# weiji14/deepbedmap

Hardware: NVIDIA B200
Metric: continent inference output Mpx/s (higher is better)
Workload: dtype bf16 (fp32 accumulate, fp32 residual stream)

## Files before the change

### deepbedmap_b200/csrc/common.cuh

```cuda
#pragma once
#include <cuda.h>
#include <cuda_bf16.h>
#include <cuda_runtime.h>
#include <stdint.h>
#include <stdio.h>

#include "../../include/deepbedmap_b200.h"

namespace dbm {

void set_error(const char* fmt, ...);
int check_launch(const char* what);

#define DBM_REQUIRE(cond, ...)            \
  do {                                    \
    if (!(cond)) {                        \
      ::dbm::set_error(__VA_ARGS__);      \
      return DBM_ERR_INVALID;             \
    }                                     \
  } while (0)

#define DBM_CUDA(expr)                                                          \
  do {                                                                          \
    cudaError_t _e = (expr);                                                    \
// ... 59 lines not shown
    if ((++spins & 1023u) != 0) return false;
    const unsigned long long now = globaltimer_ns();
    if (t0 == 0) { t0 = now; return false; }
    return now - t0 > 20000000000ull;
  }
};

__device__ __forceinline__ void mbar_wait(uint64_t* bar, uint32_t parity) {
  uint32_t spins = 0;
  while (!mbar_try_wait(bar, parity)) {
    if (++spins > (1u << 26)) {
      printf("dbm: mbarrier wait timeout block %d thread %d\n", blockIdx.x, threadIdx.x);
      __trap();
    }
  }
}

__device__ __forceinline__ void tma_prefetch_desc(const void* tmap) {
  asm volatile("prefetch.tensormap [%0];" ::"l"(tmap) : "memory");
}
__device__ __forceinline__ void tma_load_4d(void* dst, const void* tmap, uint64_t* bar, int c0, int c1,
                                            int c2, int c3) {
  asm volatile(
      "cp.async.bulk.tensor.4d.shared::cluster.global.tile.mbarrier::complete_tx::bytes "
      "[%0], [%1, {%3, %4, %5, %6}], [%2];" ::"r"(smem_u32(dst)),
      "l"(tmap), "r"(smem_u32(bar)), "r"(c0), "r"(c1), "r"(c2), "r"(c3)
      : "memory");
}
__device__ __forceinline__ void bulk_load(void* dst, const void* src, uint32_t bytes, uint64_t* bar) {
  asm volatile(
      "cp.async.bulk.shared::cluster.global.mbarrier::complete_tx::bytes [%0], [%1], %2, [%3];" ::"r"(
          smem_u32(dst)),
      "l"(src), "r"(bytes), "r"(smem_u32(bar))
      : "memory");
}

template <uint32_t kCols>
__device__ __forceinline__ void tmem_alloc(uint32_t* dst_smem) {
  asm volatile("tcgen05.alloc.cta_group::1.sync.aligned.shared::cta.b32 [%0], %1;" ::"r"(
                   smem_u32(dst_smem)),
               "n"(kCols)
               : "memory");
  asm volatile("tcgen05.relinquish_alloc_permit.cta_group::1.sync.aligned;" ::: "memory");
}
template <uint32_t kCols>
__device__ __forceinline__ void tmem_dealloc(uint32_t taddr) {
  asm volatile("tcgen05.dealloc.cta_group::1.sync.aligned.b32 %0, %1;" ::"r"(taddr), "n"(kCols)
               : "memory");
}
__device__ __forceinline__ void tc_fence_before() {
  asm volatile("tcgen05.fence::before_thread_sync;" ::: "memory");
}
__device__ __forceinline__ void tc_fence_after() {
  asm volatile("tcgen05.fence::after_thread_sync;" ::: "memory");
}
__device__ __forceinline__ void umma_bf16(uint32_t d_tmem, uint64_t adesc, uint64_t bdesc, uint32_t idesc,
                                          uint32_t accumulate) {
  asm volatile(
      "{\n\t.reg .pred p;\n\t"
      "setp.ne.b32 p, %4, 0;\n\t"
      "tcgen05.mma.cta_group::1.kind::f16 [%0], %1, %2, %3, p;\n\t}" ::"r"(d_tmem),
      "l"(adesc), "l"(bdesc), "r"(idesc), "r"(accumulate)
      : "memory");
}
template <uint32_t kAOff, uint32_t kBOff>
__device__ __forceinline__ void umma_bf16_off(uint32_t d_tmem, uint32_t a_lo, uint32_t a_hi, uint32_t b_lo,
                                              uint32_t b_hi, uint32_t idesc, uint32_t accumulate) {
  asm volatile(
      "{\n\t.reg .pred p;\n\t.reg .b32 alo, blo;\n\t.reg .b64 ad, bd;\n\t"
      "setp.ne.b32 p, %6, 0;\n\t"
      "add.u32 alo, %1, %7;\n\t"
      "add.u32 blo, %3, %8;\n\t"
      "mov.b64 ad, {alo, %2};\n\t"
      "mov.b64 bd, {blo, %4};\n\t"
      "tcgen05.mma.cta_group::1.kind::f16 [%0], ad, bd, %5, p;\n\t}" ::"r"(d_tmem),
      "r"(a_lo), "r"(a_hi), "r"(b_lo), "r"(b_hi), "r"(idesc), "r"(accumulate), "n"(kAOff), "n"(kBOff)
      : "memory");
}
__device__ __forceinline__ void umma_commit(uint64_t* bar) {
  asm volatile("tcgen05.commit.cta_group::1.mbarrier::arrive::one.shared::cluster.b64 [%0];" ::"r"(
                   smem_u32(bar))
               : "memory");
}
__device__ __forceinline__ void tmem_ld_32x32b_x32(uint32_t taddr, uint32_t (&r)[32]) {
  asm volatile(
      "tcgen05.ld.sync.aligned.32x32b.x32.b32 "
      "{%0, %1, %2, %3, %4, %5, %6, %7, %8, %9, %10, %11, %12, %13, %14, %15, "
      "%16, %17, %18, %19, %20, %21, %22, %23, %24, %25, %26, %27, %28, %29, %30, %31}, [%32];"
      : "=r"(r[0]), "=r"(r[1]), "=r"(r[2]), "=r"(r[3]), "=r"(r[4]), "=r"(r[5]), "=r"(r[6]), "=r"(r[7]),
        "=r"(r[8]), "=r"(r[9]), "=r"(r[10]), "=r"(r[11]), "=r"(r[12]), "=r"(r[13]), "=r"(r[14]),
        "=r"(r[15]), "=r"(r[16]), "=r"(r[17]), "=r"(r[18]), "=r"(r[19]), "=r"(r[20]), "=r"(r[21]),
        "=r"(r[22]), "=r"(r[23]), "=r"(r[24]), "=r"(r[25]), "=r"(r[26]), "=r"(r[27]), "=r"(r[28]),
        "=r"(r[29]), "=r"(r[30]), "=r"(r[31])
      : "r"(taddr)
      : "memory");
}
__device__ __forceinline__ void tmem_wait_ld() {
  asm volatile("tcgen05.wait::ld.sync.aligned;" ::: "memory");
}

__device__ __forceinline__ bool elect_one_sync() {
  uint32_t pred = 0;
  asm volatile(
      "{\n\t.reg .pred P1;\n\t"
      "elect.sync _|P1, 0xFFFFFFFF;\n\t"
      "@P1 mov.s32 %0, 1;\n\t}"
      : "+r"(pred));
  return pred != 0;
}
__device__ __forceinline__ uint64_t make_desc(uint32_t lo, uint32_t hi) {
  return ((uint64_t)hi << 32) | (uint64_t)lo;
}
__device__ __forceinline__ uint32_t desc_lo(uint32_t saddr, uint32_t lbo_bytes) {
  return ((saddr & 0x3FFFFu) >> 4) | (((lbo_bytes >> 4) & 0x3FFFu) << 16);
}
__host__ __device__ constexpr uint32_t desc_hi(uint32_t sbo_bytes) {
  return ((sbo_bytes >> 4) & 0x3FFFu) | (1u << 14);
}

__device__ __forceinline__ uint64_t umma_desc_kmajor_noswz(uint32_t saddr, uint32_t lbo_bytes,
                                                           uint32_t sbo_bytes) {
  uint64_t d = 0;
  d |= (uint64_t)((saddr & 0x3FFFFu) >> 4);
  d |= (uint64_t)((lbo_bytes >> 4) & 0x3FFF) << 16;
  d |= (uint64_t)((sbo_bytes >> 4) & 0x3FFF) << 32;
  d |= (uint64_t)1 << 46;
  return d;
}
__host__ __device__ constexpr uint32_t umma_idesc_bf16(uint32_t M, uint32_t N) {
  return (1u << 4) | (1u << 7) | (1u << 10) | ((N >> 3) << 17) | ((M >> 4) << 24);
}

}
```

### deepbedmap_b200/csrc/debug_bench.cu

```cuda
#include <utility>

#include "common.cuh"

namespace dbm {

template <int N, int MODE, int IDX>
__device__ __forceinline__ void rate_one(uint32_t d, uint32_t a_lo, uint32_t a_hi, uint32_t b_lo, uint32_t b_hi,
                                         uint32_t idesc) {
  constexpr int tap = IDX % 9, ks = (IDX / 9) % 2, j = IDX / 18;
  constexpr uint32_t a_off = MODE == 0   ? (uint32_t)(((2 * ks) * 18 + tap / 3) * 18 + tap % 3 + 8 * j)
                             : MODE == 1 ? (uint32_t)((2 * ks) * 128 + j * 1024)
                                         : (uint32_t)(ks * 2 + (tap % 3) * 1024);
  constexpr uint32_t b_off = MODE == 2 ? (uint32_t)(ks * 2 + (tap % 2) * (N * 8))
                                       : (uint32_t)(((tap % 3) * 4 + 2 * ks) * (N / 8) * 8);
  umma_bf16_off<a_off, b_off>(d + (uint32_t)(j * N), a_lo, a_hi, b_lo, b_hi, idesc, 1u);
}
template <int N, int MODE, int... IDX>
__device__ __forceinline__ void rate_all(uint32_t d, uint32_t a_lo, uint32_t a_hi, uint32_t b_lo, uint32_t b_hi,
                                         uint32_t idesc, std::integer_sequence<int, IDX...>) {
  (rate_one<N, MODE, IDX>(d, a_lo, a_hi, b_lo, b_hi, idesc), ...);
}

template <int N, int MODE>
__global__ void __launch_bounds__(128, 1) umma_rate_kernel(int iters, long long* out) {
  extern __shared__ uint8_t smem_raw[];
  uint8_t* smem = (uint8_t*)(((uintptr_t)smem_raw + 1023) & ~(uintptr_t)1023);
  __shared__ uint64_t bar;
  __shared__ uint32_t tmem_slot;
  for (int i = threadIdx.x; i < 160 * 1024 / 4; i += blockDim.x) ((uint32_t*)smem)[i] = 0x3c003c00u;
  if (threadIdx.x == 0) {
    mbar_init(&bar, 1);
    fence_mbar_init();
  }
  fence_proxy_async_smem();
  if (threadIdx.x < 32) tmem_alloc<512>(&tmem_slot);
  tc_fence_before();
  __syncthreads();
  tc_fence_after();
  const uint32_t tmem = tmem_slot;
  if (threadIdx.x < 32) {
    constexpr uint32_t idesc = umma_idesc_bf16(128, N);
    const uint32_t a0 = smem_u32(smem), b0 = smem_u32(smem + 96 * 1024);
    uint32_t a_lo, a_hi, b_lo, b_hi;
    if (MODE == 0) {
      a_lo = desc_lo(a0, 5184); a_hi = desc_hi(288);
      b_lo = desc_lo(b0, (N / 8) * 128); b_hi = desc_hi(128);
    } else if (MODE == 1) {
      a_lo = desc_lo(a0, 2048); a_hi = desc_hi(128);
      b_lo = desc_lo(b0, (N / 8) * 128); b_hi = desc_hi(128);
    } else {
      a_lo = desc_lo(a0, 16); a_hi = desc_hi(1024) | (2u << 29);
      b_lo = desc_lo(b0, 16); b_hi = desc_hi(1024) | (2u << 29);
    }
    uint32_t ph = 0;
    const long long t0 = clock64();
    for (int it = 0; it < iters; ++it) {
      if (elect_one_sync()) {
        rate_all<N, MODE>(tmem, a_lo, a_hi, b_lo, b_hi, idesc, std::make_integer_sequence<int, 36>{});
        umma_commit(&bar);
      }
      __syncwarp();
      mbar_wait(&bar, ph);
      ph ^= 1;
    }
    const long long t1 = clock64();
    if (threadIdx.x == 0) out[blockIdx.x] = t1 - t0;
  }
  tc_fence_before();
  __syncthreads();
  if (threadIdx.x < 32) {
    tc_fence_after();
    tmem_dealloc<512>(tmem);
  }
}

template <int N, int MODE>
static int launch_rate(int iters, long long* out, int grid, cudaStream_t st) {
  const int smem = 160 * 1024 + 2048;
  DBM_CUDA(cudaFuncSetAttribute(umma_rate_kernel<N, MODE>, cudaFuncAttributeMaxDynamicSharedMemorySize, smem));
  umma_rate_kernel<N, MODE><<<grid, 128, smem, st>>>(iters, out);
  return check_launch("umma_rate_kernel");
}

}

using namespace dbm;

extern "C" int dbm_debug_umma_rate(int mode, int n, int iters, int per_commit, long long* out_cycles, int grid,
                                   cudaStream_t stream) {
  (void)per_commit;
#define DBM_RATE(NN)                                                         \
  if (n == NN) {                                                             \
    if (mode == 0) return launch_rate<NN, 0>(iters, out_cycles, grid, stream); \
    if (mode == 1) return launch_rate<NN, 1>(iters, out_cycles, grid, stream); \
    if (mode == 2) return launch_rate<NN, 2>(iters, out_cycles, grid, stream); \
  }
  DBM_RATE(32) DBM_RATE(64) DBM_RATE(128) DBM_RATE(256)
#undef DBM_RATE
  set_error("umma_rate: unsupported n=%d mode=%d", n, mode);
  return DBM_ERR_INVALID;
}
```

### deepbedmap_b200/csrc/umma_trunk.cu

```cuda
#include "umma_common.cuh"

namespace dbm {

constexpr int kTrunkThreads = 320;
constexpr int kEpiWarps = 8;
constexpr int kTW = 16, kTH = 32;
constexpr int kHW = kTW + 2, kHH = kTH + 2;
constexpr int kTStages = 5;
constexpr int kTABytes = kHW * kHH * 16 * 2;
constexpr int kTBBytesMax = 9 * 16 * 64 * 2;
constexpr int kMaxTrunkLayers = 512;
constexpr int kTrunkSmem = kTStages * (kTABytes + kTBBytesMax) + 256 + kMaxTrunkLayers * 28 + kEpiWarps * 256 + 1024;

struct TrunkMaps {
  CUtensorMap m[3];
};

template <int COUT>
__device__ __forceinline__ void issue_stage_wide(uint32_t d0, uint32_t a_lo, uint32_t a_hi, uint32_t b_lo,
                                                 uint32_t b_hi, uint32_t acc0) {
  constexpr uint32_t idesc = umma_idesc_bf16(128, COUT);
  constexpr uint32_t kBTap = (uint32_t)(2 * (COUT / 8) * 8);
#pragma unroll 1
  for (uint32_t tap = 0; tap < 9; ++tap) {
    const uint32_t a_tap = a_lo + tap + (tap / 3) * (kHW - 3);
    const uint32_t b_tap = b_lo + tap * kBTap;
    const uint32_t acc = tap != 0 ? 1u : acc0;
    umma_bf16_off<0, 0>(d0, a_tap, a_hi, b_tap, b_hi, idesc, acc);
    umma_bf16_off<8, 0>(d0 + 64, a_tap, a_hi, b_tap, b_hi, idesc, acc);
    umma_bf16_off<16 * kHW, 0>(d0 + 128, a_tap, a_hi, b_tap, b_hi, idesc, acc);
    umma_bf16_off<16 * kHW + 8, 0>(d0 + 192, a_tap, a_hi, b_tap, b_hi, idesc, acc);
  }
}

extern int g_trunk_debug;
extern unsigned long long* g_trunk_prof;

struct TrunkParams {
  const TrunkLayer* layers;
  int num_layers;
  int N, H, W, tiles_x, tiles_y, items_per_layer;
  unsigned int* done;
  unsigned long long* prof;
  int debug;
};

__device__ __forceinline__ unsigned int ld_relaxed_gpu(const unsigned int* p) {
  unsigned int v;
  asm volatile("ld.relaxed.gpu.global.u32 %0, [%1];" : "=r"(v) : "l"(p) : "memory");
  return v;
}
__device__ __forceinline__ void fence_acq_rel_gpu() { asm volatile("fence.acq_rel.gpu;" ::: "memory"); }
__device__ __forceinline__ unsigned int ld_acquire_gpu(const unsigned int* p) {
  unsigned int v;
  asm volatile("ld.acquire.gpu.global.u32 %0, [%1];" : "=r"(v) : "l"(p) : "memory");
  return v;
}
struct F8 {
  float v[8];
};
__device__ __forceinline__ F8 ld_cg_f8(const float* p) {
  F8 r;
  asm volatile("ld.global.cg.v8.f32 {%0,%1,%2,%3,%4,%5,%6,%7}, [%8];"
               : "=f"(r.v[0]), "=f"(r.v[1]), "=f"(r.v[2]), "=f"(r.v[3]), "=f"(r.v[4]), "=f"(r.v[5]), "=f"(r.v[6]),
                 "=f"(r.v[7])
               : "l"(p)
               : "memory");
  return r;
}
__device__ __forceinline__ void st_f8(float* p, float a0, float a1, float a2, float a3, float a4, float a5, float a6,
                                      float a7) {
  asm volatile("st.global.v8.f32 [%0], {%1,%2,%3,%4,%5,%6,%7,%8};" ::"l"(p), "f"(a0), "f"(a1), "f"(a2), "f"(a3),
               "f"(a4), "f"(a5), "f"(a6), "f"(a7)
               : "memory");
}

__device__ __forceinline__ void split_bf16x8(const float* v, uint4& hi, uint4& lo) {
  uint32_t h[4], l[4];
#pragma unroll
  for (int i = 0; i < 4; ++i) {
    const __nv_bfloat162 t = __floats2bfloat162_rn(v[2 * i], v[2 * i + 1]);
    const float2 f = __bfloat1622float2(t);
    const __nv_bfloat162 u = __floats2bfloat162_rn(v[2 * i] - f.x, v[2 * i + 1] - f.y);
    h[i] = *reinterpret_cast<const uint32_t*>(&t);
    l[i] = *reinterpret_cast<const uint32_t*>(&u);
  }
  hi = make_uint4(h[0], h[1], h[2], h[3]);
  lo = make_uint4(l[0], l[1], l[2], l[3]);
}
__device__ __forceinline__ int split_slab(int L) { return ((L >> 1) << 2) + (L & 1); }

struct Cursor {
  int grp = 0, step = 0;
};
struct Sched {
  const int* groups;
  int ng, I, Gd, rounds, bid;
  __device__ __forceinline__ bool next(Cursor& c, int& L, int& unit, int& buf) const {
    while (c.grp < ng) {
      const int e = groups[c.grp];
      const bool pair = (e >> 30) & 1;
      const int nsteps = pair ? 2 * rounds : rounds;
      if (c.step >= nsteps) {
        ++c.grp;
        c.step = 0;
        continue;
      }
      const int t = c.step++;
      int round = t, tail = 0;
      if (pair) {
        if (t == 0) round = 0;
        else if (t == nsteps - 1) { round = rounds - 1; tail = 1; }
        else if (t & 1) round = (t + 1) >> 1;
        else { round = (t >> 1) - 1; tail = 1; }
      }
      int r = bid - (int)(((long)c.grp * I) % Gd);
      if (r < 0) r += Gd;
      unit = round * Gd + r;
      if (unit >= I) continue;
      L = (e & 0x3FFFFFFF) + tail;
      buf = round & 1;
      return true;
    }
    return false;
  }
};

template <bool SPLIT>
__global__ void __launch_bounds__(kTrunkThreads, 1)
umma_trunk_kernel(const __grid_constant__ TrunkMaps maps, const TrunkParams p) {
  extern __shared__ uint8_t smem_raw[];
  uint8_t* smem = (uint8_t*)(((uintptr_t)smem_raw + 1023) & ~(uintptr_t)1023);
  uint8_t* smA = smem;
  uint8_t* smB = smem + kTStages * kTABytes;
  uint64_t* bars = (uint64_t*)(smem + kTStages * (kTABytes + kTBBytesMax));
  uint64_t* full = bars;
  uint64_t* empty = bars + kTStages;
  uint64_t* tfull = bars + 2 * kTStages;
  uint64_t* tempty = bars + 2 * kTStages + 2;
  uint32_t* tmem_slot = (uint32_t*)(bars + 2 * kTStages + 4);
  int* ng_slot = (int*)(tmem_slot + 1);
  int4* linfo = (int4*)(smem + kTStages * (kTABytes + kTBBytesMax) + 256);
  const __nv_bfloat16** lw = (const __nv_bfloat16**)(linfo + kMaxTrunkLayers);
  float* sbias_all = (float*)(lw + kMaxTrunkLayers);
  int* groups = (int*)(sbias_all + kEpiWarps * 64);

  const int warp = threadIdx.x >> 5;
  const int lane = threadIdx.x & 31;

  for (int L = threadIdx.x; L < p.num_layers; L += kTrunkThreads) {
    const TrunkLayer* ly = p.layers + L;
    linfo[L] = make_int4(ly->cin, ly->cout, ly->in_map | (ly->mode << 8), ly->in_cs0);
    lw[L] = ly->wpacked;
  }
  if (threadIdx.x == 0) {
    int ng = 0;
    for (int L = 0; L < p.num_layers; ++L) {
      const int mode = p.layers[L].mode;
      const bool ok = mode == 0 || (mode == 1 && p.layers[L].cout == 64 && L + 1 < p.num_layers &&
                                    p.layers[L + 1].mode == 2 && p.layers[L + 1].cout == 32) ||
                      (mode == 2 && L > 0 && p.layers[L - 1].mode == 1);
      if (!ok) {
        if (blockIdx.x == 0) printf("dbm: trunk pass table entry %d: bad pairing (mode %d)\n", L, mode);
        __trap();
      }
      if (mode == 2) continue;
      groups[ng++] = L | (mode == 1 ? (1 << 30) : 0);
    }
    *ng_slot = ng;
  }
  if (warp == 0 && lane == 0) {
    for (int i = 0; i < 3; ++i) tma_prefetch_desc(&maps.m[i]);
    for (int s = 0; s < kTStages; ++s) {
      mbar_init(&full[s], 1);
      mbar_init(&empty[s], 1);
    }
    for (int b = 0; b < 2; ++b) {
      mbar_init(&tfull[b], 1);
      mbar_init(&tempty[b], kEpiWarps / 2);
    }
    fence_mbar_init();
  }
  if (warp == 1) tmem_alloc<512>(tmem_slot);
  tc_fence_before();
  __syncthreads();
  tc_fence_after();
  const uint32_t tmem_base = *tmem_slot;

  const int I = p.items_per_layer;
  const int per_img = p.tiles_x * p.tiles_y;
  Sched sc;
  sc.groups = groups; sc.ng = *ng_slot; sc.I = I; sc.Gd = (int)gridDim.x; sc.bid = (int)blockIdx.x;
  sc.rounds = (I + sc.Gd - 1) / sc.Gd;
  const unsigned int need = (unsigned)(kEpiWarps / 2);

  if (warp == 0) {
    int s = 0;
    uint32_t ph = 0;
    auto flag_of = [&](int L, int unit) -> const unsigned int* {
      if (L == 0 || lane >= 9) return nullptr;
      const int n = unit / per_img;
      const int r = unit - n * per_img;
      const int ty = r / p.tiles_x, tx = r - ty * p.tiles_x;
      const int ny = ty + lane / 3 - 1, nx = tx + lane % 3 - 1;
      if (ny < 0 || ny >= p.tiles_y || nx < 0 || nx >= p.tiles_x) return nullptr;
      return p.done + (size_t)(L - 1) * I + (size_t)n * per_img + ny * p.tiles_x + nx;
    };
    Cursor cur;
    int L, unit, buf;
    bool have = sc.next(cur, L, unit, buf);
    const unsigned int* f_cur = have ? flag_of(L, unit) : nullptr;
    unsigned int v_cur = f_cur != nullptr ? ld_relaxed_gpu(f_cur) : need;
    while (have) {
      const int n = unit / per_img;
      const int r = unit - n * per_img;
      const int ty = r / p.tiles_x, tx = r - ty * p.tiles_x;
      const int4 li = linfo[L];
      const int cin = li.x, cout = li.y, in_map = li.z & 0xFF, in_cs0 = li.w;
      const __nv_bfloat16* wp = lw[L];
      if (L > 0 && !(p.debug & 1)) {
        if (f_cur != nullptr) {
          SpinGuard guard;
          while (v_cur < need) {
            if (guard.expired()) {
              printf("dbm: trunk dependency timeout layer %d unit %d\n", L, unit);
              __trap();
            }
            __nanosleep(64);
            v_cur = ld_relaxed_gpu(f_cur);
          }
        }
        __syncwarp();
        fence_acq_rel_gpu();
      }
      int Ln, unitn, bufn;
      have = sc.next(cur, Ln, unitn, bufn);
      f_cur = have ? flag_of(Ln, unitn) : nullptr;
      v_cur = f_cur != nullptr ? ld_relaxed_gpu(f_cur) : need;
      const CUtensorMap* tm = &maps.m[in_map];
      const uint32_t b_bytes = (uint32_t)(9 * 16 * 2) * (uint32_t)cout;
      const int num_kc = SPLIT ? 3 * (cin >> 4) : (cin >> 4);
      for (int kc = 0; kc < num_kc; ++kc) {
        int slab = in_cs0 + kc * 2;
        if constexpr (SPLIT) {
          const int c16 = kc / 3, t = kc - 3 * c16;
          slab = 2 * in_cs0 + 4 * c16 + (t == 1 ? 2 : 0);
        }
        mbar_wait(&empty[s], ph ^ 1);
        if (elect_one_sync()) {
          if (p.debug & 4) {
            mbar_arrive(&full[s]);
          } else {
            asm volatile("fence.proxy.async.global;" ::: "memory");
            mbar_arrive_expect_tx(&full[s], (uint32_t)kTABytes + b_bytes);
            tma_load_4d(smA + s * kTABytes, tm, &full[s], (tx * kTW - 1) * 8, ty * kTH - 1, slab,
                        (p.debug & 256) ? 0 : n);
            bulk_load(smB + s * kTBBytesMax, wp + (size_t)kc * (b_bytes / 2), b_bytes, &full[s]);
          }
        }
        __syncwarp();
        if (++s == kTStages) { s = 0; ph ^= 1; }
      }
      L = Ln; unit = unitn; buf = bufn;
    }
  } else if (warp == 1) {
    const uint32_t a_hi = desc_hi(kHW * 16);
    const uint32_t b_hi = desc_hi(128);
    const uint32_t smA_u = smem_u32(smA), smB_u = smem_u32(smB);
    int s = 0;
    uint32_t ph = 0;
    uint32_t use[2] = {0, 0};
    Cursor cur;
    int L, unit, buf;
    while (sc.next(cur, L, unit, buf)) {
      const int4 li = linfo[L];
      const int cin = li.x, cout = li.y, mode = li.z >> 8;
      const int num_kc = SPLIT ? 3 * (cin >> 4) : (cin >> 4);
      const long long t0 = p.prof ? clock64() : 0;
      mbar_wait(&tempty[buf], (use[buf] & 1) ^ 1);
      ++use[buf];
      tc_fence_after();
      const long long t1 = p.prof ? clock64() : 0;
      long long tw = 0;
      const uint32_t d0 = tmem_base + (uint32_t)(buf * 256 + (mode == 2 ? 32 : 0));
      for (int kc = 0; kc < num_kc; ++kc) {
        const long long tw0 = p.prof ? clock64() : 0;
        mbar_wait(&full[s], ph);
        tc_fence_after();
        if (p.prof) tw += clock64() - tw0;
        const uint32_t a_lo = desc_lo(smA_u + s * kTABytes, kHW * kHH * 16);
        const uint32_t acc0 = (kc != 0 || mode == 2) ? 1u : 0u;
        if (cout == 32) {
          const uint32_t b_lo = desc_lo(smB_u + s * kTBBytesMax, 4 * 128);
          if (elect_one_sync()) {
            issue_stage_wide<32>(d0, a_lo, a_hi, b_lo, b_hi, acc0);
            umma_commit(&empty[s]);
            if (kc == num_kc - 1) umma_commit(&tfull[buf]);
          }
        } else {
          const uint32_t b_lo = desc_lo(smB_u + s * kTBBytesMax, 8 * 128);
          if (elect_one_sync()) {
            issue_stage_wide<64>(d0, a_lo, a_hi, b_lo, b_hi, acc0);
            umma_commit(&empty[s]);
            if (kc == num_kc - 1) umma_commit(&tfull[buf]);
          }
        }
        __syncwarp();
        if (++s == kTStages) { s = 0; ph ^= 1; }
      }
      if (p.prof && lane == 0) {
        atomicAdd(p.prof + L * 8 + 0, (unsigned long long)(t1 - t0));
        atomicAdd(p.prof + L * 8 + 1, (unsigned long long)tw);
        atomicAdd(p.prof + L * 8 + 2, (unsigned long long)(clock64() - t0));
        atomicAdd(p.prof + L * 8 + 3, 1ull);
      }
    }
  } else {
    const int q = warp & 3;
    const int grp = (warp - 2) >> 2;
    const int m = 32 * q + lane;
    const int gy = m >> 3, xr = m & 7;
    const bool mem = !(p.debug & 2);
    const bool mem_f32 = mem && !(p.debug & 32), mem_bf16 = mem && !(p.debug & 64), mem_res = mem && !(p.debug & 128);
    const size_t plane = (size_t)p.H * p.W;
    float* sbias = sbias_all + (warp - 2) * 64;
    uint32_t use = 0;
    Cursor cur;
    int L, item, buf;
    while (sc.next(cur, L, item, buf)) {
      if (buf != grp) continue;
      const int n_img = item / per_img;
      const int r = item - n_img * per_img;
      const int n = (p.debug & 256) ? 0 : n_img;
      const int ty = r / p.tiles_x, tx = r - ty * p.tiles_x;
      const TrunkLayer ly = p.layers[L];
      const int y0 = ty * kTH + gy;
      const int x0 = tx * kTW + xr;
      const int nbc = ly.mode == 0 ? (ly.cout >> 5) : 1;
      const int col_off = ly.mode == 2 ? 32 : 0;
      const int nblk = 4 * nbc;
      const int cmain = nbc << 5;
      F8 r1[4], r1n[4];
      if (lane < cmain) sbias[lane] = __ldg(ly.bias + lane);
      if (lane + 32 < cmain) sbias[lane + 32] = __ldg(ly.bias + lane + 32);
      if (L > 0 && (ly.res1 || ly.res2) && !(p.debug & 1)) {
        if (lane == 0) {
          const unsigned int* f = p.done + (size_t)(L - 1) * I + item;
          SpinGuard guard;
          while (ld_acquire_gpu(f) < need) {
            if (guard.expired()) {
              printf("dbm: trunk epilogue dependency timeout layer %d item %d\n", L, item);
              __trap();
            }
            __nanosleep(32);
          }
        }
      }
      __syncwarp();
      auto load_r1 = [&](int b, F8 (&dst)[4]) {
        const int j = nbc == 2 ? (b >> 1) : b;
        const int c0 = (b - j * nbc) << 5;
        const int x = x0 + 8 * (j & 1), y = y0 + 16 * (j >> 1);
        if (ly.res1 != nullptr && mem_res && y < p.H && x < p.W) {
          const float* rp =
              ly.res1 + (((size_t)n * (ly.res1_cs_total >> 1) + (c0 >> 3)) * plane + (size_t)y * p.W + x) * 8;
#pragma unroll
          for (int s8 = 0; s8 < 4; ++s8) dst[s8] = ld_cg_f8(rp + (size_t)s8 * plane * 8);
        }
      };
      load_r1(0, r1);
      const long long e0 = p.prof ? clock64() : 0;
      mbar_wait(&tfull[grp], use & 1);
      ++use;
      tc_fence_after();
      const long long e1 = p.prof ? clock64() : 0;
      long long e2 = 0;
      const bool quick = nbc == 1 && ly.res1 == nullptr && ly.res2 == nullptr && ly.out_f32 == nullptr && !ly.up2 &&
                         ly.out_bf16 != nullptr;
      if (quick) {
        const uint32_t tb = tmem_base + ((uint32_t)(32 * q) << 16) + (uint32_t)(grp * 256 + col_off);
#pragma unroll
        for (int half = 0; half < 2; ++half) {
          uint32_t acc2[2][32];
          tmem_ld_32x32b_x32(tb + (uint32_t)((2 * half) * 64), acc2[0]);
          tmem_ld_32x32b_x32(tb + (uint32_t)((2 * half + 1) * 64), acc2[1]);
          tmem_wait_ld();
          if (half == 1) {
            tc_fence_before();
            __syncwarp();
            if (lane == 0) mbar_arrive(&tempty[grp]);
            if (p.prof) e2 = clock64();
          }
#pragma unroll
          for (int jj = 0; jj < 2; ++jj) {
            const int x = x0 + 8 * jj;
            const int y = y0 + 16 * half;
            if (y < p.H && x < p.W && mem_bf16) {
              const size_t pix = (size_t)y * p.W + x;
#pragma unroll
              for (int s8 = 0; s8 < 4; ++s8) {
                const float4 ba = *reinterpret_cast<const float4*>(sbias + 8 * s8);
                const float4 bb = *reinterpret_cast<const float4*>(sbias + 8 * s8 + 4);
                float v[8] = {__uint_as_float(acc2[jj][8 * s8 + 0]) + ba.x, __uint_as_float(acc2[jj][8 * s8 + 1]) + ba.y,
                              __uint_as_float(acc2[jj][8 * s8 + 2]) + ba.z, __uint_as_float(acc2[jj][8 * s8 + 3]) + ba.w,
                              __uint_as_float(acc2[jj][8 * s8 + 4]) + bb.x, __uint_as_float(acc2[jj][8 * s8 + 5]) + bb.y,
                              __uint_as_float(acc2[jj][8 * s8 + 6]) + bb.z, __uint_as_float(acc2[jj][8 * s8 + 7]) + bb.w};
                if (ly.act) {
#pragma unroll
                  for (int i = 0; i < 8; ++i) v[i] = lrelu(v[i]);
                }
                if constexpr (SPLIT) {
                  uint4 hi, lo;
                  split_bf16x8(v, hi, lo);
                  const size_t cs = (size_t)n * (2 * ly.out_cs_total) + split_slab(ly.out_cs0 + s8);
                  *reinterpret_cast<uint4*>(ly.out_bf16 + (cs * plane + pix) * 8) = hi;
                  *reinterpret_cast<uint4*>(ly.out_bf16 + ((cs + 2) * plane + pix) * 8) = lo;
                  continue;
                }
                uint4 o;
                __nv_bfloat162 t0 = __floats2bfloat162_rn(v[0], v[1]);
                __nv_bfloat162 t1 = __floats2bfloat162_rn(v[2], v[3]);
                __nv_bfloat162 t2 = __floats2bfloat162_rn(v[4], v[5]);
                __nv_bfloat162 t3 = __floats2bfloat162_rn(v[6], v[7]);
                o.x = *reinterpret_cast<uint32_t*>(&t0);
                o.y = *reinterpret_cast<uint32_t*>(&t1);
                o.z = *reinterpret_cast<uint32_t*>(&t2);
                o.w = *reinterpret_cast<uint32_t*>(&t3);
                const size_t cs = (size_t)n * ly.out_cs_total + (ly.out_cs0 + s8);
                *reinterpret_cast<uint4*>(ly.out_bf16 + (cs * plane + pix) * 8) = o;
              }
            }
          }
        }
      } else
      for (int b = 0; b < nblk; ++b) {
        const int j = nbc == 2 ? (b >> 1) : b;
        const int c0 = (b - j * nbc) << 5;
        const int x = x0 + 8 * (j & 1);
        const int y = y0 + 16 * (j >> 1);
        const bool valid = (y < p.H) && (x < p.W);
        const size_t pix = (size_t)y * p.W + x;
        uint32_t acc[32];
        tmem_ld_32x32b_x32(tmem_base + ((uint32_t)(32 * q) << 16) + (uint32_t)(grp * 256 + j * 64 + col_off + c0), acc);
        const bool has1 = ly.res1 != nullptr && valid && mem_res, has2 = ly.res2 != nullptr && valid && mem_res;
        if (b + 1 < nblk) load_r1(b + 1, r1n);
        tmem_wait_ld();
        if (b == nblk - 1) {
          tc_fence_before();
          __syncwarp();
          if (lane == 0) mbar_arrive(&tempty[grp]);
          if (p.prof) e2 = clock64();
        }
        if (valid) {
        float v[32];
#pragma unroll
        for (int i4 = 0; i4 < 8; ++i4) {
          const float4 bb = *reinterpret_cast<const float4*>(sbias + c0 + 4 * i4);
          v[4 * i4 + 0] = __uint_as_float(acc[4 * i4 + 0]) + bb.x;
          v[4 * i4 + 1] = __uint_as_float(acc[4 * i4 + 1]) + bb.y;
          v[4 * i4 + 2] = __uint_as_float(acc[4 * i4 + 2]) + bb.z;
          v[4 * i4 + 3] = __uint_as_float(acc[4 * i4 + 3]) + bb.w;
        }
        if (has1) {
#pragma unroll
          for (int i = 0; i < 32; ++i) v[i] = r1[i >> 3].v[i & 7] + ly.beta * v[i];
        }
        if (has2) {
          const float* rp = ly.res2 + (((size_t)n * 8 + (c0 >> 3)) * plane + pix) * 8;
#pragma unroll
          for (int s8 = 0; s8 < 4; ++s8) {
            const F8 rr = ld_cg_f8(rp + (size_t)s8 * plane * 8);
#pragma unroll
            for (int i = 0; i < 8; ++i) v[8 * s8 + i] = rr.v[i] + ly.beta * v[8 * s8 + i];
          }
        }
        if (ly.act) {
#pragma unroll
          for (int i = 0; i < 32; ++i) v[i] = lrelu(v[i]);
        }
        if (ly.out_f32 && mem_f32) {
          float* op = ly.out_f32 + (((size_t)n * 8 + (c0 >> 3)) * plane + pix) * 8;
#pragma unroll
          for (int s8 = 0; s8 < 4; ++s8)
            st_f8(op + (size_t)s8 * plane * 8, v[8 * s8], v[8 * s8 + 1], v[8 * s8 + 2], v[8 * s8 + 3], v[8 * s8 + 4],
                  v[8 * s8 + 5], v[8 * s8 + 6], v[8 * s8 + 7]);
        }
        if (ly.out_bf16 && mem_bf16) {
#pragma unroll
          for (int s8 = 0; s8 < 4; ++s8) {
            uint4 o, o_lo = make_uint4(0, 0, 0, 0);
            size_t cs;
            if constexpr (SPLIT) {
              split_bf16x8(v + 8 * s8, o, o_lo);
              cs = (size_t)n * (2 * ly.out_cs_total) + split_slab(ly.out_cs0 + c0 / 8 + s8);
            } else {
              __nv_bfloat162 t0 = __floats2bfloat162_rn(v[8 * s8 + 0], v[8 * s8 + 1]);
              __nv_bfloat162 t1 = __floats2bfloat162_rn(v[8 * s8 + 2], v[8 * s8 + 3]);
              __nv_bfloat162 t2 = __floats2bfloat162_rn(v[8 * s8 + 4], v[8 * s8 + 5]);
              __nv_bfloat162 t3 = __floats2bfloat162_rn(v[8 * s8 + 6], v[8 * s8 + 7]);
              o.x = *reinterpret_cast<uint32_t*>(&t0);
              o.y = *reinterpret_cast<uint32_t*>(&t1);
              o.z = *reinterpret_cast<uint32_t*>(&t2);
              o.w = *reinterpret_cast<uint32_t*>(&t3);
              cs = (size_t)n * ly.out_cs_total + (ly.out_cs0 + c0 / 8 + s8);
            }
#pragma unroll 1
            for (int part = 0; part < (SPLIT ? 2 : 1); ++part) {
              const uint4 ov = part ? o_lo : o;
              const size_t csp = cs + 2 * part;
              if (!ly.up2) {
                *reinterpret_cast<uint4*>(ly.out_bf16 + (csp * plane + pix) * 8) = ov;
              } else {
                const int Ho = 2 * p.H, Wo = 2 * p.W;
                __nv_bfloat16* base = ly.out_bf16 + ((csp * Ho + 2 * y) * Wo + 2 * x) * 8;
                *reinterpret_cast<uint4*>(base) = ov;
                *reinterpret_cast<uint4*>(base + 8) = ov;
                *reinterpret_cast<uint4*>(base + (size_t)Wo * 8) = ov;
                *reinterpret_cast<uint4*>(base + (size_t)Wo * 8 + 8) = ov;
              }
            }
          }
        }
        }
#pragma unroll
        for (int s8 = 0; s8 < 4; ++s8) r1[s8] = r1n[s8];
      }
      if (p.debug & 8) __threadfence();
      __syncwarp();
      if (lane == 0) {
        if (!(p.debug & 16)) __threadfence();
        atomicAdd(p.done + (size_t)L * I + item, 1u);
        if (p.prof && q == 0) {
          atomicAdd(p.prof + L * 8 + 4, (unsigned long long)(e1 - e0));
          atomicAdd(p.prof + L * 8 + 5, (unsigned long long)(e2 - e1));
          atomicAdd(p.prof + L * 8 + 6, (unsigned long long)(clock64() - e2));
        }
      }
    }
  }

  tc_fence_before();
  __syncthreads();
  if (warp == 1) {
    tc_fence_after();
    tmem_dealloc<512>(tmem_base);
  }
}

}

using namespace dbm;

namespace dbm {
int g_trunk_debug = 0;
unsigned long long* g_trunk_prof = nullptr;
}

extern "C" int dbm_debug_set_ptr(int key, void* ptr) {
  if (key == 1) g_trunk_prof = (unsigned long long*)ptr;
  return DBM_OK;
}

static int trunk_umma_launch(const void* layers_dev, int num_layers, int n, int h, int w, const void* stem_slab8,
                             int stem_cs_total, const void* cat_a_slab8, const void* cat_b_slab8, int cat_cs_total,
                             unsigned int* flags_dev, int split, cudaStream_t stream) {
  DBM_REQUIRE(num_layers > 0 && n > 0 && h > 0 && w > 0, "trunk: empty problem");
  DBM_REQUIRE(num_layers <= kMaxTrunkLayers, "trunk: %d passes exceed the kernel's table of %d", num_layers,
              kMaxTrunkLayers);
  DBM_REQUIRE(((uintptr_t)layers_dev & 7) == 0, "trunk: layer table must be 8-byte aligned");
  TrunkMaps maps;
  const void* bases[3] = {stem_slab8, cat_a_slab8, cat_b_slab8};
  const int cs_tot[3] = {stem_cs_total << split, cat_cs_total << split, cat_cs_total << split};
  for (int i = 0; i < 3; ++i) {
    int rc = make_slab8_tmap(&maps.m[i], bases[i], n, cs_tot[i], h, w, 16, kHW, kHH);
    if (rc) return rc;
  }
  TrunkParams p;
  p.layers = (const TrunkLayer*)layers_dev;
  p.num_layers = num_layers;
  p.N = n; p.H = h; p.W = w;
  p.tiles_x = ceil_div(w, kTW); p.tiles_y = ceil_div(h, kTH);
  p.items_per_layer = n * p.tiles_x * p.tiles_y;
  p.done = flags_dev;
  p.debug = g_trunk_debug;
  p.prof = g_trunk_prof;
  DBM_CUDA(cudaMemsetAsync(flags_dev, 0, (size_t)num_layers * p.items_per_layer * sizeof(unsigned int), stream));
  const long total = p.items_per_layer;
  int resident = 0;
  const void* kfn = split ? (const void*)umma_trunk_kernel<true> : (const void*)umma_trunk_kernel<false>;
  int rc2 = resident_ctas(kfn, kTrunkThreads, kTrunkSmem, &resident);
  if (rc2) return rc2;
  const int grid = total < resident ? (int)total : resident;
  if (split)
    umma_trunk_kernel<true><<<grid, kTrunkThreads, kTrunkSmem, stream>>>(maps, p);
  else
    umma_trunk_kernel<false><<<grid, kTrunkThreads, kTrunkSmem, stream>>>(maps, p);
  return check_launch("umma_trunk_kernel");
}

extern "C" int dbm_trunk_umma(const void* layers_dev, int num_layers, int n, int h, int w, const void* stem_slab8,
                              int stem_cs_total, const void* cat_a_slab8, const void* cat_b_slab8, int cat_cs_total,
                              unsigned int* flags_dev, cudaStream_t stream) {
  return trunk_umma_launch(layers_dev, num_layers, n, h, w, stem_slab8, stem_cs_total, cat_a_slab8, cat_b_slab8,
                           cat_cs_total, flags_dev, 0, stream);
}

extern "C" int dbm_trunk_umma_split(const void* layers_dev, int num_layers, int n, int h, int w,
                                    const void* stem_slab8, int stem_cs_total, const void* cat_a_slab8,
                                    const void* cat_b_slab8, int cat_cs_total, unsigned int* flags_dev,
                                    cudaStream_t stream) {
  return trunk_umma_launch(layers_dev, num_layers, n, h, w, stem_slab8, stem_cs_total, cat_a_slab8, cat_b_slab8,
                           cat_cs_total, flags_dev, 1, stream);
}
```

Baseline: 328.2.

## Run trunk convolution as 2-CTA cluster UMMA with split weight loads

Converts the persistent trunk conv kernel to 2-CTA clusters using cta_group::2 tcgen05 MMA with M=256. Each CTA in a pair handles an adjacent x-tile and loads half of the weight slab, so per-CTA weight traffic and smem are halved. The freed smem allows more pipeline stages. The leader issues MMAs for both CTAs, with cross-CTA mbarrier signalling for full and tmem-empty. It adds cluster sync overhead and wastes work on padded odd tiles. It also adds a 2-CTA rate microbenchmark mode.

Result: no change. 327.4, median of 6 (-0.3%).

```diff
diff --git a/deepbedmap_b200/csrc/common.cuh b/deepbedmap_b200/csrc/common.cuh
--- a/deepbedmap_b200/csrc/common.cuh
+++ b/deepbedmap_b200/csrc/common.cuh
@@ -165,6 +165,76 @@
                    smem_u32(bar))
                : "memory");
 }
+__device__ __forceinline__ uint32_t cluster_ctarank() {
+  uint32_t r;
+  asm volatile("mov.u32 %0, %%cluster_ctarank;" : "=r"(r));
+  return r;
+}
+__device__ __forceinline__ uint32_t cluster_id_x() {
+  uint32_t r;
+  asm volatile("mov.u32 %0, %%clusterid.x;" : "=r"(r));
+  return r;
+}
+__device__ __forceinline__ void cluster_sync_all() {
+  asm volatile("barrier.cluster.arrive.release.aligned;\n\tbarrier.cluster.wait.acquire.aligned;" ::: "memory");
+}
+__device__ __forceinline__ uint32_t mapa_shared(const void* p, uint32_t rank) {
+  uint32_t r;
+  asm volatile("mapa.shared::cluster.u32 %0, %1, %2;" : "=r"(r) : "r"(smem_u32(p)), "r"(rank));
+  return r;
+}
+__device__ __forceinline__ void mbar_arrive_cluster(uint32_t cluster_addr) {
+  asm volatile("mbarrier.arrive.release.cluster.shared::cluster.b64 _, [%0];" ::"r"(cluster_addr) : "memory");
+}
+__device__ __forceinline__ void mbar_wait_cluster(uint64_t* bar, uint32_t parity) {
+  uint32_t spins = 0;
+  for (;;) {
+    uint32_t ok;
+    asm volatile(
+        "{\n\t.reg .pred p;\n\t"
+        "mbarrier.try_wait.parity.acquire.cluster.shared::cta.b64 p, [%1], %2;\n\t"
+        "selp.u32 %0, 1, 0, p;\n\t}"
+        : "=r"(ok)
+        : "r"(smem_u32(bar)), "r"(parity)
+        : "memory");
+    if (ok) return;
+    if (++spins > (1u << 26)) {
+      printf("dbm: mbarrier wait timeout block %d thread %d\n", blockIdx.x, threadIdx.x);
+      __trap();
+    }
+  }
+}
+template <uint32_t kCols>
+__device__ __forceinline__ void tmem_alloc2(uint32_t* dst_smem) {
+  asm volatile("tcgen05.alloc.cta_group::2.sync.aligned.shared::cta.b32 [%0], %1;" ::"r"(smem_u32(dst_smem)),
+               "n"(kCols)
+               : "memory");
+  asm volatile("tcgen05.relinquish_alloc_permit.cta_group::2.sync.aligned;" ::: "memory");
+}
+template <uint32_t kCols>
+__device__ __forceinline__ void tmem_dealloc2(uint32_t taddr) {
+  asm volatile("tcgen05.dealloc.cta_group::2.sync.aligned.b32 %0, %1;" ::"r"(taddr), "n"(kCols) : "memory");
+}
+template <uint32_t kAOff, uint32_t kBOff>
+__device__ __forceinline__ void umma2_bf16_off(uint32_t d_tmem, uint32_t a_lo, uint32_t a_hi, uint32_t b_lo,
+                                               uint32_t b_hi, uint32_t idesc, uint32_t accumulate) {
+  asm volatile(
+      "{\n\t.reg .pred p;\n\t.reg .b32 alo, blo;\n\t.reg .b64 ad, bd;\n\t"
+      "setp.ne.b32 p, %6, 0;\n\t"
+      "add.u32 alo, %1, %7;\n\t"
+      "add.u32 blo, %3, %8;\n\t"
+      "mov.b64 ad, {alo, %2};\n\t"
+      "mov.b64 bd, {blo, %4};\n\t"
+      "tcgen05.mma.cta_group::2.kind::f16 [%0], ad, bd, %5, p;\n\t}" ::"r"(d_tmem),
+      "r"(a_lo), "r"(a_hi), "r"(b_lo), "r"(b_hi), "r"(idesc), "r"(accumulate), "n"(kAOff), "n"(kBOff)
+      : "memory");
+}
+__device__ __forceinline__ void umma2_commit_both(uint64_t* bar) {
+  asm volatile("tcgen05.commit.cta_group::2.mbarrier::arrive::one.shared::cluster.multicast::cluster.b64 [%0], %1;" ::
+                   "r"(smem_u32(bar)), "h"((uint16_t)3)
+               : "memory");
+}
+
 __device__ __forceinline__ void tmem_ld_32x32b_x32(uint32_t taddr, uint32_t (&r)[32]) {
   asm volatile(
       "tcgen05.ld.sync.aligned.32x32b.x32.b32 "
diff --git a/deepbedmap_b200/csrc/debug_bench.cu b/deepbedmap_b200/csrc/debug_bench.cu
--- a/deepbedmap_b200/csrc/debug_bench.cu
+++ b/deepbedmap_b200/csrc/debug_bench.cu
@@ -74,12 +74,83 @@
   }
 }
 
+template <int N, int IDX>
+__device__ __forceinline__ void rate2_one(uint32_t d, uint32_t a_lo, uint32_t a_hi, uint32_t b_lo, uint32_t b_hi,
+                                          uint32_t idesc) {
+  constexpr int tap = IDX % 9, ks = (IDX / 9) % 2, j = IDX / 18;
+  constexpr uint32_t a_off = (uint32_t)(((2 * ks) * 18 + tap / 3) * 18 + tap % 3 + 8 * j);
+  constexpr uint32_t b_off = (uint32_t)(((tap % 3) * 4 + 2 * ks) * (N / 16) * 8);
+  umma2_bf16_off<a_off, b_off>(d + (uint32_t)(j * N), a_lo, a_hi, b_lo, b_hi, idesc, 1u);
+}
+template <int N, int... IDX>
+__device__ __forceinline__ void rate2_all(uint32_t d, uint32_t a_lo, uint32_t a_hi, uint32_t b_lo, uint32_t b_hi,
+                                          uint32_t idesc, std::integer_sequence<int, IDX...>) {
+  (rate2_one<N, IDX>(d, a_lo, a_hi, b_lo, b_hi, idesc), ...);
+}
+
+template <int N>
+__global__ void __cluster_dims__(2, 1, 1) __launch_bounds__(128, 1) umma_rate2_kernel(int iters, long long* out) {
+  extern __shared__ uint8_t smem_raw[];
+  uint8_t* smem = (uint8_t*)(((uintptr_t)smem_raw + 1023) & ~(uintptr_t)1023);
+  __shared__ uint64_t bar;
+  __shared__ uint32_t tmem_slot;
+  const bool leader = cluster_ctarank() == 0;
+  for (int i = threadIdx.x; i < 160 * 1024 / 4; i += blockDim.x) ((uint32_t*)smem)[i] = 0x3c003c00u;
+  if (threadIdx.x == 0) {
+    mbar_init(&bar, 1);
+    fence_mbar_init();
+  }
+  fence_proxy_async_smem();
+  if (threadIdx.x < 32) {
+    tmem_alloc2<512>(&tmem_slot);
+  }
+  tc_fence_before();
+  cluster_sync_all();
+  tc_fence_after();
+  const uint32_t tmem = tmem_slot;
+  if (leader && threadIdx.x < 32) {
+    constexpr uint32_t idesc = umma_idesc_bf16(256, N);
+    const uint32_t a0 = smem_u32(smem), b0 = smem_u32(smem + 96 * 1024);
+    const uint32_t a_lo = desc_lo(a0, 5184), a_hi = desc_hi(288);
+    const uint32_t b_lo = desc_lo(b0, (N / 16) * 128), b_hi = desc_hi(128);
+    uint32_t ph = 0;
+    const long long t0 = clock64();
+    for (int it = 0; it < iters; ++it) {
+      if (elect_one_sync()) {
+        rate2_all<N>(tmem, a_lo, a_hi, b_lo, b_hi, idesc, std::make_integer_sequence<int, 36>{});
+        asm volatile("tcgen05.commit.cta_group::2.mbarrier::arrive::one.shared::cluster.b64 [%0];" ::"r"(
+                         smem_u32(&bar))
+                     : "memory");
+      }
+      __syncwarp();
+      mbar_wait(&bar, ph);
+      ph ^= 1;
+    }
+    const long long t1 = clock64();
+    if (threadIdx.x == 0) out[blockIdx.x] = t1 - t0;
+  }
+  if (!leader && threadIdx.x == 0) out[blockIdx.x] = 0;
+  tc_fence_before();
+  cluster_sync_all();
+  if (threadIdx.x < 32) {
+    tc_fence_after();
+    tmem_dealloc2<512>(tmem);
+  }
+}
+
 template <int N, int MODE>
 static int launch_rate(int iters, long long* out, int grid, cudaStream_t st) {
   const int smem = 160 * 1024 + 2048;
-  DBM_CUDA(cudaFuncSetAttribute(umma_rate_kernel<N, MODE>, cudaFuncAttributeMaxDynamicSharedMemorySize, smem));
-  umma_rate_kernel<N, MODE><<<grid, 128, smem, st>>>(iters, out);
-  return check_launch("umma_rate_kernel");
+  if constexpr (MODE == 3) {
+    DBM_REQUIRE(grid % 2 == 0, "umma_rate: mode 3 runs 2-CTA clusters, grid %d is odd", grid);
+    DBM_CUDA(cudaFuncSetAttribute(umma_rate2_kernel<N>, cudaFuncAttributeMaxDynamicSharedMemorySize, smem));
+    umma_rate2_kernel<N><<<grid, 128, smem, st>>>(iters, out);
+    return check_launch("umma_rate2_kernel");
+  } else {
+    DBM_CUDA(cudaFuncSetAttribute(umma_rate_kernel<N, MODE>, cudaFuncAttributeMaxDynamicSharedMemorySize, smem));
+    umma_rate_kernel<N, MODE><<<grid, 128, smem, st>>>(iters, out);
+    return check_launch("umma_rate_kernel");
+  }
 }
 
 }
@@ -94,6 +165,7 @@
     if (mode == 0) return launch_rate<NN, 0>(iters, out_cycles, grid, stream); \
     if (mode == 1) return launch_rate<NN, 1>(iters, out_cycles, grid, stream); \
     if (mode == 2) return launch_rate<NN, 2>(iters, out_cycles, grid, stream); \
+    if (mode == 3) return launch_rate<NN, 3>(iters, out_cycles, grid, stream); \
   }
   DBM_RATE(32) DBM_RATE(64) DBM_RATE(128) DBM_RATE(256)
 #undef DBM_RATE
diff --git a/deepbedmap_b200/csrc/umma_trunk.cu b/deepbedmap_b200/csrc/umma_trunk.cu
--- a/deepbedmap_b200/csrc/umma_trunk.cu
+++ b/deepbedmap_b200/csrc/umma_trunk.cu
@@ -6,9 +6,9 @@
 constexpr int kEpiWarps = 8;
 constexpr int kTW = 16, kTH = 32;
 constexpr int kHW = kTW + 2, kHH = kTH + 2;
-constexpr int kTStages = 5;
+constexpr int kTStages = 7;
 constexpr int kTABytes = kHW * kHH * 16 * 2;
-constexpr int kTBBytesMax = 9 * 16 * 64 * 2;
+constexpr int kTBBytesMax = 9 * 16 * 32 * 2;
 constexpr int kMaxTrunkLayers = 512;
 constexpr int kTrunkSmem = kTStages * (kTABytes + kTBBytesMax) + 256 + kMaxTrunkLayers * 28 + kEpiWarps * 256 + 1024;
 
@@ -19,17 +19,17 @@
 template <int COUT>
 __device__ __forceinline__ void issue_stage_wide(uint32_t d0, uint32_t a_lo, uint32_t a_hi, uint32_t b_lo,
                                                  uint32_t b_hi, uint32_t acc0) {
-  constexpr uint32_t idesc = umma_idesc_bf16(128, COUT);
-  constexpr uint32_t kBTap = (uint32_t)(2 * (COUT / 8) * 8);
+  constexpr uint32_t idesc = umma_idesc_bf16(256, COUT);
+  constexpr uint32_t kBTap = (uint32_t)(2 * (COUT / 16) * 8);
 #pragma unroll 1
   for (uint32_t tap = 0; tap < 9; ++tap) {
     const uint32_t a_tap = a_lo + tap + (tap / 3) * (kHW - 3);
     const uint32_t b_tap = b_lo + tap * kBTap;
     const uint32_t acc = tap != 0 ? 1u : acc0;
-    umma_bf16_off<0, 0>(d0, a_tap, a_hi, b_tap, b_hi, idesc, acc);
-    umma_bf16_off<8, 0>(d0 + 64, a_tap, a_hi, b_tap, b_hi, idesc, acc);
-    umma_bf16_off<16 * kHW, 0>(d0 + 128, a_tap, a_hi, b_tap, b_hi, idesc, acc);
-    umma_bf16_off<16 * kHW + 8, 0>(d0 + 192, a_tap, a_hi, b_tap, b_hi, idesc, acc);
+    umma2_bf16_off<0, 0>(d0, a_tap, a_hi, b_tap, b_hi, idesc, acc);
+    umma2_bf16_off<8, 0>(d0 + 64, a_tap, a_hi, b_tap, b_hi, idesc, acc);
+    umma2_bf16_off<16 * kHW, 0>(d0 + 128, a_tap, a_hi, b_tap, b_hi, idesc, acc);
+    umma2_bf16_off<16 * kHW + 8, 0>(d0 + 192, a_tap, a_hi, b_tap, b_hi, idesc, acc);
   }
 }
 
@@ -40,6 +40,7 @@
   const TrunkLayer* layers;
   int num_layers;
   int N, H, W, tiles_x, tiles_y, items_per_layer;
+  int pairs_x, pairs_per_layer;
   unsigned int* done;
   unsigned long long* prof;
   int debug;
@@ -147,6 +148,8 @@
 
   const int warp = threadIdx.x >> 5;
   const int lane = threadIdx.x & 31;
+  const uint32_t rank = cluster_ctarank();
+  const int nclusters = (int)(gridDim.x >> 1);
 
   for (int L = threadIdx.x; L < p.num_layers; L += kTrunkThreads) {
     const TrunkLayer* ly = p.layers + L;
@@ -172,36 +175,43 @@
   if (warp == 0 && lane == 0) {
     for (int i = 0; i < 3; ++i) tma_prefetch_desc(&maps.m[i]);
     for (int s = 0; s < kTStages; ++s) {
-      mbar_init(&full[s], 1);
+      mbar_init(&full[s], rank == 0 ? 2 : 1);
       mbar_init(&empty[s], 1);
     }
     for (int b = 0; b < 2; ++b) {
       mbar_init(&tfull[b], 1);
-      mbar_init(&tempty[b], kEpiWarps / 2);
+      mbar_init(&tempty[b], kEpiWarps);
     }
     fence_mbar_init();
   }
-  if (warp == 1) tmem_alloc<512>(tmem_slot);
+  if (warp == 1) tmem_alloc2<512>(tmem_slot);
   tc_fence_before();
-  __syncthreads();
+  cluster_sync_all();
   tc_fence_after();
   const uint32_t tmem_base = *tmem_slot;
 
   const int I = p.items_per_layer;
   const int per_img = p.tiles_x * p.tiles_y;
+  const int per_img_pairs = p.pairs_x * p.tiles_y;
   Sched sc;
-  sc.groups = groups; sc.ng = *ng_slot; sc.I = I; sc.Gd = (int)gridDim.x; sc.bid = (int)blockIdx.x;
-  sc.rounds = (I + sc.Gd - 1) / sc.Gd;
+  sc.groups = groups; sc.ng = *ng_slot; sc.I = p.pairs_per_layer; sc.Gd = nclusters; sc.bid = (int)cluster_id_x();
+  sc.rounds = (sc.I + sc.Gd - 1) / sc.Gd;
   const unsigned int need = (unsigned)(kEpiWarps / 2);
+  auto unit_of = [&](int pr, int& n, int& ty, int& tx) {
+    n = pr / per_img_pairs;
+    const int r = pr - n * per_img_pairs;
+    ty = r / p.pairs_x;
+    tx = 2 * (r - ty * p.pairs_x) + (int)rank;
+  };
 
   if (warp == 0) {
     int s = 0;
     uint32_t ph = 0;
-    auto flag_of = [&](int L, int unit) -> const unsigned int* {
+    auto flag_of = [&](int L, int pr) -> const unsigned int* {
       if (L == 0 || lane >= 9) return nullptr;
-      const int n = unit / per_img;
-      const int r = unit - n * per_img;
-      const int ty = r / p.tiles_x, tx = r - ty * p.tiles_x;
+      int n, ty, tx;
+      unit_of(pr, n, ty, tx);
+      if (tx >= p.tiles_x) return nullptr;
       const int ny = ty + lane / 3 - 1, nx = tx + lane % 3 - 1;
       if (ny < 0 || ny >= p.tiles_y || nx < 0 || nx >= p.tiles_x) return nullptr;
       return p.done + (size_t)(L - 1) * I + (size_t)n * per_img + ny * p.tiles_x + nx;
@@ -212,9 +222,8 @@
     const unsigned int* f_cur = have ? flag_of(L, unit) : nullptr;
     unsigned int v_cur = f_cur != nullptr ? ld_relaxed_gpu(f_cur) : need;
     while (have) {
-      const int n = unit / per_img;
-      const int r = unit - n * per_img;
-      const int ty = r / p.tiles_x, tx = r - ty * p.tiles_x;
+      int n, ty, tx;
+      unit_of(unit, n, ty, tx);
       const int4 li = linfo[L];
       const int cin = li.x, cout = li.y, in_map = li.z & 0xFF, in_cs0 = li.w;
       const __nv_bfloat16* wp = lw[L];
@@ -239,6 +248,7 @@
       v_cur = f_cur != nullptr ? ld_relaxed_gpu(f_cur) : need;
       const CUtensorMap* tm = &maps.m[in_map];
       const uint32_t b_bytes = (uint32_t)(9 * 16 * 2) * (uint32_t)cout;
+      const uint32_t run = 8u * (uint32_t)cout;
       const int num_kc = SPLIT ? 3 * (cin >> 4) : (cin >> 4);
       for (int kc = 0; kc < num_kc; ++kc) {
         int slab = in_cs0 + kc * 2;
@@ -247,21 +257,41 @@
           slab = 2 * in_cs0 + 4 * c16 + (t == 1 ? 2 : 0);
         }
         mbar_wait(&empty[s], ph ^ 1);
-        if (elect_one_sync()) {
-          if (p.debug & 4) {
-            mbar_arrive(&full[s]);
-          } else {
+        if (p.debug & 4) {
+          if (elect_one_sync()) mbar_arrive(&full[s]);
+        } else {
+          if (elect_one_sync()) {
             asm volatile("fence.proxy.async.global;" ::: "memory");
-            mbar_arrive_expect_tx(&full[s], (uint32_t)kTABytes + b_bytes);
+            mbar_arrive_expect_tx(&full[s], (uint32_t)kTABytes + b_bytes / 2);
             tma_load_4d(smA + s * kTABytes, tm, &full[s], (tx * kTW - 1) * 8, ty * kTH - 1, slab,
                         (p.debug & 256) ? 0 : n);
-            bulk_load(smB + s * kTBBytesMax, wp + (size_t)kc * (b_bytes / 2), b_bytes, &full[s]);
+          }
+          __syncwarp();
+          if (lane < 18) {
+            const uint8_t* src = (const uint8_t*)(wp + (size_t)kc * (b_bytes / 2)) + (lane * 2u + rank) * run;
+            bulk_load(smB + s * kTBBytesMax + lane * run, src, run, &full[s]);
           }
         }
         __syncwarp();
         if (++s == kTStages) { s = 0; ph ^= 1; }
       }
       L = Ln; unit = unitn; buf = bufn;
+    }
+  } else if (warp == 1 && rank == 1) {
+    const uint32_t full0 = mapa_shared(full, 0);
+    int s = 0;
+    uint32_t ph = 0;
+    Cursor cur;
+    int L, unit, buf;
+    while (sc.next(cur, L, unit, buf)) {
+      const int cin = linfo[L].x;
+      const int num_kc = SPLIT ? 3 * (cin >> 4) : (cin >> 4);
+      for (int kc = 0; kc < num_kc; ++kc) {
+        mbar_wait(&full[s], ph);
+        if (lane == 0) mbar_arrive_cluster(full0 + 8u * (uint32_t)s);
+        __syncwarp();
+        if (++s == kTStages) { s = 0; ph ^= 1; }
+      }
     }
   } else if (warp == 1) {
     const uint32_t a_hi = desc_hi(kHW * 16);
@@ -277,7 +307,7 @@
       const int cin = li.x, cout = li.y, mode = li.z >> 8;
       const int num_kc = SPLIT ? 3 * (cin >> 4) : (cin >> 4);
       const long long t0 = p.prof ? clock64() : 0;
-      mbar_wait(&tempty[buf], (use[buf] & 1) ^ 1);
+      mbar_wait_cluster(&tempty[buf], (use[buf] & 1) ^ 1);
       ++use[buf];
       tc_fence_after();
       const long long t1 = p.prof ? clock64() : 0;
@@ -285,24 +315,24 @@
       const uint32_t d0 = tmem_base + (uint32_t)(buf * 256 + (mode == 2 ? 32 : 0));
       for (int kc = 0; kc < num_kc; ++kc) {
         const long long tw0 = p.prof ? clock64() : 0;
-        mbar_wait(&full[s], ph);
+        mbar_wait_cluster(&full[s], ph);
         tc_fence_after();
         if (p.prof) tw += clock64() - tw0;
         const uint32_t a_lo = desc_lo(smA_u + s * kTABytes, kHW * kHH * 16);
         const uint32_t acc0 = (kc != 0 || mode == 2) ? 1u : 0u;
         if (cout == 32) {
+          const uint32_t b_lo = desc_lo(smB_u + s * kTBBytesMax, 2 * 128);
+          if (elect_one_sync()) {
+            issue_stage_wide<32>(d0, a_lo, a_hi, b_lo, b_hi, acc0);
+            umma2_commit_both(&empty[s]);
+            if (kc == num_kc - 1) umma2_commit_both(&tfull[buf]);
+          }
+        } else {
           const uint32_t b_lo = desc_lo(smB_u + s * kTBBytesMax, 4 * 128);
           if (elect_one_sync()) {
-            issue_stage_wide<32>(d0, a_lo, a_hi, b_lo, b_hi, acc0);
-            umma_commit(&empty[s]);
-            if (kc == num_kc - 1) umma_commit(&tfull[buf]);
-          }
-        } else {
-          const uint32_t b_lo = desc_lo(smB_u + s * kTBBytesMax, 8 * 128);
-          if (elect_one_sync()) {
             issue_stage_wide<64>(d0, a_lo, a_hi, b_lo, b_hi, acc0);
-            umma_commit(&empty[s]);
-            if (kc == num_kc - 1) umma_commit(&tfull[buf]);
+            umma2_commit_both(&empty[s]);
+            if (kc == num_kc - 1) umma2_commit_both(&tfull[buf]);
           }
         }
         __syncwarp();
@@ -324,15 +354,17 @@
     const bool mem_f32 = mem && !(p.debug & 32), mem_bf16 = mem && !(p.debug & 64), mem_res = mem && !(p.debug & 128);
     const size_t plane = (size_t)p.H * p.W;
     float* sbias = sbias_all + (warp - 2) * 64;
+    const uint32_t tempty0 = mapa_shared(tempty, 0);
     uint32_t use = 0;
     Cursor cur;
-    int L, item, buf;
-    while (sc.next(cur, L, item, buf)) {
+    int L, pr, buf;
+    while (sc.next(cur, L, pr, buf)) {
       if (buf != grp) continue;
-      const int n_img = item / per_img;
-      const int r = item - n_img * per_img;
+      int n_img, ty, tx;
+      unit_of(pr, n_img, ty, tx);
+      const bool real = tx < p.tiles_x;
+      const int item = n_img * per_img + ty * p.tiles_x + tx;
       const int n = (p.debug & 256) ? 0 : n_img;
-      const int ty = r / p.tiles_x, tx = r - ty * p.tiles_x;
       const TrunkLayer ly = p.layers[L];
       const int y0 = ty * kTH + gy;
       const int x0 = tx * kTW + xr;
@@ -343,7 +375,7 @@
       F8 r1[4], r1n[4];
       if (lane < cmain) sbias[lane] = __ldg(ly.bias + lane);
       if (lane + 32 < cmain) sbias[lane + 32] = __ldg(ly.bias + lane + 32);
-      if (L > 0 && (ly.res1 || ly.res2) && !(p.debug & 1)) {
+      if (L > 0 && (ly.res1 || ly.res2) && !(p.debug & 1) && real) {
         if (lane == 0) {
           const unsigned int* f = p.done + (size_t)(L - 1) * I + item;
           SpinGuard guard;
@@ -388,7 +420,7 @@
           if (half == 1) {
             tc_fence_before();
             __syncwarp();
-            if (lane == 0) mbar_arrive(&tempty[grp]);
+            if (lane == 0) mbar_arrive_cluster(tempty0 + 8u * (uint32_t)grp);
             if (p.prof) e2 = clock64();
           }
 #pragma unroll
@@ -448,7 +480,7 @@
         if (b == nblk - 1) {
           tc_fence_before();
           __syncwarp();
-          if (lane == 0) mbar_arrive(&tempty[grp]);
+          if (lane == 0) mbar_arrive_cluster(tempty0 + 8u * (uint32_t)grp);
           if (p.prof) e2 = clock64();
         }
         if (valid) {
@@ -527,10 +559,10 @@
       }
       if (p.debug & 8) __threadfence();
       __syncwarp();
-      if (lane == 0) {
+      if (lane == 0 && real) {
         if (!(p.debug & 16)) __threadfence();
         atomicAdd(p.done + (size_t)L * I + item, 1u);
-        if (p.prof && q == 0) {
+        if (p.prof && q == 0 && rank == 0) {
           atomicAdd(p.prof + L * 8 + 4, (unsigned long long)(e1 - e0));
           atomicAdd(p.prof + L * 8 + 5, (unsigned long long)(e2 - e1));
           atomicAdd(p.prof + L * 8 + 6, (unsigned long long)(clock64() - e2));
@@ -540,10 +572,10 @@
   }
 
   tc_fence_before();
-  __syncthreads();
+  cluster_sync_all();
   if (warp == 1) {
     tc_fence_after();
-    tmem_dealloc<512>(tmem_base);
+    tmem_dealloc2<512>(tmem_base);
   }
 }
 
@@ -558,6 +590,37 @@
 
 extern "C" int dbm_debug_set_ptr(int key, void* ptr) {
   if (key == 1) g_trunk_prof = (unsigned long long*)ptr;
+  return DBM_OK;
+}
+
+static int resident_trunk_clusters(const void* kernel, int* clusters) {
+  struct Entry { int dev; const void* k; int value; };
+  static Entry cache[16];
+  static int used = 0;
+  int dev = 0;
+  DBM_CUDA(cudaGetDevice(&dev));
+  for (int i = 0; i < used; ++i)
+    if (cache[i].dev == dev && cache[i].k == kernel) {
+      *clusters = cache[i].value;
+      return DBM_OK;
+    }
+  DBM_CUDA(cudaFuncSetAttribute(kernel, cudaFuncAttributeMaxDynamicSharedMemorySize, kTrunkSmem));
+  cudaLaunchConfig_t cfg = {};
+  cudaLaunchAttribute attr[1];
+  attr[0].id = cudaLaunchAttributeClusterDimension;
+  attr[0].val.clusterDim.x = 2;
+  attr[0].val.clusterDim.y = 1;
+  attr[0].val.clusterDim.z = 1;
+  cfg.gridDim = dim3(2);
+  cfg.blockDim = dim3(kTrunkThreads);
+  cfg.dynamicSmemBytes = kTrunkSmem;
+  cfg.attrs = attr;
+  cfg.numAttrs = 1;
+  int n = 0;
+  DBM_CUDA(cudaOccupancyMaxActiveClusters(&n, kernel, &cfg));
+  DBM_REQUIRE(n >= 1, "trunk kernel: not one 2-CTA cluster can be resident (%d B shared memory per CTA)", kTrunkSmem);
+  *clusters = n;
+  if (used < 16) cache[used++] = Entry{dev, kernel, n};
   return DBM_OK;
 }
 
@@ -581,20 +644,34 @@
   p.N = n; p.H = h; p.W = w;
   p.tiles_x = ceil_div(w, kTW); p.tiles_y = ceil_div(h, kTH);
   p.items_per_layer = n * p.tiles_x * p.tiles_y;
+  p.pairs_x = (p.tiles_x + 1) / 2;
+  p.pairs_per_layer = n * p.pairs_x * p.tiles_y;
   p.done = flags_dev;
   p.debug = g_trunk_debug;
   p.prof = g_trunk_prof;
   DBM_CUDA(cudaMemsetAsync(flags_dev, 0, (size_t)num_layers * p.items_per_layer * sizeof(unsigned int), stream));
-  const long total = p.items_per_layer;
+  const long total = p.pairs_per_layer;
   int resident = 0;
   const void* kfn = split ? (const void*)umma_trunk_kernel<true> : (const void*)umma_trunk_kernel<false>;
-  int rc2 = resident_ctas(kfn, kTrunkThreads, kTrunkSmem, &resident);
+  int rc2 = resident_trunk_clusters(kfn, &resident);
   if (rc2) return rc2;
-  const int grid = total < resident ? (int)total : resident;
+  const int clusters = total < resident ? (int)total : resident;
+  cudaLaunchConfig_t cfg = {};
+  cudaLaunchAttribute attr[1];
+  attr[0].id = cudaLaunchAttributeClusterDimension;
+  attr[0].val.clusterDim.x = 2;
+  attr[0].val.clusterDim.y = 1;
+  attr[0].val.clusterDim.z = 1;
+  cfg.gridDim = dim3(2 * clusters);
+  cfg.blockDim = dim3(kTrunkThreads);
+  cfg.dynamicSmemBytes = kTrunkSmem;
+  cfg.stream = stream;
+  cfg.attrs = attr;
+  cfg.numAttrs = 1;
   if (split)
-    umma_trunk_kernel<true><<<grid, kTrunkThreads, kTrunkSmem, stream>>>(maps, p);
+    DBM_CUDA(cudaLaunchKernelEx(&cfg, umma_trunk_kernel<true>, maps, p));
   else
-    umma_trunk_kernel<false><<<grid, kTrunkThreads, kTrunkSmem, stream>>>(maps, p);
+    DBM_CUDA(cudaLaunchKernelEx(&cfg, umma_trunk_kernel<false>, maps, p));
   return check_launch("umma_trunk_kernel");
 }
 
```
